# AlainSchoebi/semantic-bundle-adjustment-colmap

Hardware: AMD Instinct MI355X
Metric: residuals+Jacobians/sec and BA-iteration wall-time, 1k cams / 1M pts / 10M obs (higher is better)
Workload: dtype f64

## Files before the change

### semantic-bundle-adjustment-colmap_amd/csrc/context.h

```cpp
#pragma once

#include <hip/hip_runtime.h>
#include <rocblas/rocblas.h>
#include <rccl/rccl.h>

#include <map>
#include <string>
#include <vector>

#include "../../include/mi_ba.h"
#include "cholesky.h"
#include "device.h"
#include "setup.h"

namespace miba {

template <typename T>
struct DevArray {
  T* ptr = nullptr;
  size_t n = 0;
  size_t cap = 0;
  DevArray() = default;
  DevArray(const DevArray&) = delete;
  DevArray& operator=(const DevArray&) = delete;
  ~DevArray() { release(); }
  hipError_t alloc(size_t count) {
    if (ptr && count <= cap) {
      n = count;
      return hipSuccess;
    }
    release();
    n = count;
    if (count == 0) return hipSuccess;
    const hipError_t e = hipMalloc(&ptr, sizeof(T) * count);
    if (e == hipSuccess) cap = count;
    else ptr = nullptr;
    return e;
  }
  void release() {
    if (ptr) (void)hipFree(ptr);
    ptr = nullptr;
    n = 0;
    cap = 0;
  }
  size_t bytes() const { return sizeof(T) * n; }
};

struct SemanticState;
struct GsbaState;

struct KernelTimer {
  std::vector<std::pair<std::string, std::pair<hipEvent_t, hipEvent_t>>> pending;
  std::vector<hipEvent_t> pool;
  std::vector<hipEvent_t> borrowed;
  std::map<std::string, std::pair<double, int64_t>> totals;
};

}

struct mi_ba_context {
  mi_ba_options options;
  mi_ba_problem problem;
  miba::HostSetup setup;
  miba::DevProblem dev;
  hipStream_t stream = nullptr;
  int device = 0;

  std::vector<int64_t> block_obs;
  miba::DevArray<double2> obs_xy;
  miba::DevArray<uint32_t> obs_img, obs_pt;
  miba::DevArray<uint32_t> obs_ids, wave_pt0;
  miba::DevArray<uint32_t> img_flags, img_cam;
  miba::DevArray<uint8_t> cam_var, cam_model, pt_var;
  miba::DevArray<double> qt, cam, X;
  miba::DevArray<double> qt_c, cam_c, X_c;
  miba::DevArray<double> img_rec;
  miba::DevArray<uint32_t> cm_perm;
  miba::DevArray<uint32_t> cm_ptv;
  miba::DevArray<miba::DevTile> tiles;
  int ntiles = 0;
  miba::DevArray<uint32_t> img_tile_off, cam_tile_off, cam_tiles;
  miba::DevArray<double> tpart;
  bool det_sums = true;
  const miba::TileOwners* owners() const { return det_sums && tpart.ptr ? &owners_ : nullptr; }
  miba::TileOwners owners_{};
  miba::DevArray<miba::DevPoint> vpoints;
  int64_t npv = 0;
  int64_t nb_const = 0;
  miba::DevArray<uint32_t> pchunks;
  int npchunks = 0;
  miba::DevArray<double> sum_ws;
  int lin_overlap = 0;
  int lin_warm = 15;
  int lin_warm_conc = 0;
  int warm_unroll = 4;
  int warm_wgs = 2048;
  int lin_order = 0;
  hipStream_t lin_side = nullptr;
  hipEvent_t lin_ev[2] = {nullptr, nullptr};
  int sem_diag = 0;
  bool sem_deferred_box = false;
  int sem_prep_early = 0;
  int sem_dgrid = 24;
  int sem_dvar = 0;
  int sem_compact = 1;
  int sem_coarse = 2;
  int sem_variant = 6;

  miba::DevArray<double2> r;
  miba::DevArray<double> J;
  miba::DevArray<double> Jcm;
  bool jcm_stale = true;
  miba::DevArray<double> Vg;
  miba::DevArray<double> partial;
  int64_t npartial = 0;
  miba::DevArray<double> scale_p, diag_p, Vinv;
  miba::DevArray<double> pose_blk, cam_blk, bvec, udiag;
  miba::DevArray<double> scale_f, diag_f, lambda_f, prec_pose, prec_cam;
  miba::DevArray<double> cg_x, cg_r, cg_z, cg_p, cg_q, cg_w, dX;
  miba::DevArray<double> scalars;
  miba::DevArray<double> red;
  miba::DevArray<double> aux;
  double* host_scalars = nullptr;
  int32_t* host_info = nullptr;
  int host_info_cap = 0;
  bool chol_pending = false;
  int chol_leaves = 0;

  bool dense = false;
  rocblas_handle blas = nullptr;
  miba::DevArray<double> S;
  miba::DevArray<double> Linv, Z;
  miba::DevArray<miba::DevPairTile> ptiles;
  miba::DevArray<miba::DevPairTile> ptiles_blk;
  std::vector<miba::DevPairTile> ptiles_host;
  miba::DevArray<miba::DevPairTile> ptiles_xcd;
  int nptiles_xcd = 0;
  int schur_block = 8;
  miba::DevArray<int32_t> pslot;
  miba::DevArray<double> spart;
  miba::DevArray<uint4> pdest;
  miba::DevArray<uint8_t> pself;
  int npdest = 0;
  bool pflush_ok = false;
  miba::DevArray<uint4> podest, pochunk;
  miba::DevArray<uint32_t> poent;
  miba::DevArray<double> popart;
  int npodest = 0, npochunk = 0;
  miba::DevArray<uint2> pairs;
  miba::DevArray<uint2> pairs_pos;
  int nptiles = 0;
  miba::DevArray<int32_t> info;
  miba::CholConfig chol;
  bool fused_rhs = true;
  bool pcg_mf = false;
  miba::DevArray<double> Xcm;
  miba::DevArray<double2> obs_cm;
  bool xcm_stale = true;
  int pcg_jcm = 2;
  bool pn_chunks = true;
  bool pp_chunks = true;
  bool schur_overlap = false;
  hipStream_t lm_side = nullptr;
  hipEvent_t lm_ev[2] = {nullptr, nullptr};
  miba::CholWorkspace cholws;

  double fixed_cost = 0.0;
  miba::SemanticState* sem = nullptr;
  miba::GsbaState* gsba = nullptr;

  bool timing = false;
  miba::KernelTimer timer;
  bool solved = false;

  int rank = 0, world = 1;
  ncclComm_t comm = nullptr;
  bool comm_failed = false;
  int comm_timeout_ms = 300000;
  double comm_due = 0.0;
  int fail_factorizations = 0;
  int comm_stall_ms = 0;
  int* stall_flag = nullptr;
  mi_ba_host_allreduce_fn host_reduce = nullptr;
  void* host_reduce_user = nullptr;
  std::vector<double> reduce_buf;
  bool distributed() const { return world > 1 || comm != nullptr || comm_failed || host_reduce != nullptr; }
// ... 16 lines not shown
```

### semantic-bundle-adjustment-colmap_amd/csrc/runtime.hip

```cpp
#include <hip/hip_runtime.h>

#include <algorithm>
#include <atomic>
#include <chrono>
#include <condition_variable>
#include <memory>
#include <mutex>
#include <thread>
#include <cmath>
#include <cstdio>
#include <cstring>
#include <cstdlib>
#include <map>
#include <numeric>
#include <unordered_map>

#include "../../include/mi_ba.h"
#include "ba_math.h"
#include "cholesky.h"
#include "context.h"
#include "kernels.h"
#include "gsba.h"
#include "semantic.h"
#include "setup.h"
// ... 2018 lines not shown
  bool ok;
  {
    std::unique_lock<std::mutex> g(job->m);
    job->cv.wait_for(g, std::chrono::milliseconds(std::max(1, ctx->comm_timeout_ms)), [&] { return job->done; });
    ok = job->done && job->res == ncclSuccess && job->comm;
    if (!job->done) job->abandoned = true;
    if (ok) ctx->comm = job->comm;
  }
  if (!ok) return MI_BA_ERR_HIP;
  ctx->rank = rank;
  ctx->world = world;
  return reduce_fixed_cost(ctx);
}

mi_ba_status mi_ba_context_set_host_reducer(mi_ba_context* ctx, int32_t rank, int32_t world,
                                            mi_ba_host_allreduce_fn fn, void* user) {
  if (!ctx || !fn || world < 1 || rank < 0 || rank >= world) return MI_BA_ERR_INVALID_ARGUMENT;
  if (ctx->comm || ctx->host_reduce || ctx->solved) return MI_BA_ERR_STATE;
  ctx->host_reduce = fn;
  ctx->host_reduce_user = user;
  ctx->rank = rank;
  ctx->world = world;
  return reduce_fixed_cost(ctx);
}

#ifdef MI_BA_AB_VARIANTS
static bool ab_value(int, int) { return true; }
#else
static bool ab_value(int value, int product) { return value == product; }
#endif

mi_ba_status mi_ba_set_tuning(mi_ba_context* ctx, const char* key, int32_t value) {
  if (!ctx || !key) return MI_BA_ERR_INVALID_ARGUMENT;
  if (std::strcmp(key, "jacobian_variant") == 0 && value >= 0 && value <= 63 && ab_value(value, 0)) {
    ctx->dev.jvariant = value;
    return MI_BA_OK;
  }
  if (std::strcmp(key, "comm_timeout_ms") == 0 && value >= 1) {
    ctx->comm_timeout_ms = value;
    return MI_BA_OK;
  }
  if (std::strcmp(key, "test_fail_factorizations") == 0 && value >= 0 && value <= 1000) {
    ctx->fail_factorizations = value;
    return MI_BA_OK;
  }
  if (std::strcmp(key, "comm_stall_ms") == 0 && value >= 0 && value <= 60000) {
    ctx->comm_stall_ms = value;
    return MI_BA_OK;
  }
  if (std::strcmp(key, "linearize_warm_inputs") == 0 && value >= 0 && value <= 15) {
    ctx->lin_warm = value;
    return MI_BA_OK;
  }
  if (std::strcmp(key, "linearize_warm_concurrent") == 0 && value >= 0 && value <= 15 && ab_value(value, 0)) {
    ctx->lin_warm_conc = value;
    return MI_BA_OK;
  }
  if (std::strcmp(key, "warm_unroll") == 0 && (value == 4 || value == 8) && ab_value(value, 4)) {
    ctx->warm_unroll = value;
    return MI_BA_OK;
  }
  if (std::strcmp(key, "warm_workgroups") == 0 && value >= 0 && value <= 65536) {
    ctx->warm_wgs = value;
    return MI_BA_OK;
  }
  if (std::strcmp(key, "linearize_order") == 0 && (value == 0 || value == 1) && ab_value(value, 0)) {
    ctx->lin_order = value;
    return MI_BA_OK;
  }
  if (std::strcmp(key, "linearize_overlap") == 0 && value >= 0 && value <= 2 && ab_value(value, 0)) {
    ctx->lin_overlap = value;
    return MI_BA_OK;
  }
  if (std::strcmp(key, "semantic_prep_early") == 0 && (value == 0 || value == 1) && ab_value(value, 0)) {
    ctx->sem_prep_early = value;
    return MI_BA_OK;
  }
  if (std::strcmp(key, "semantic_deferred_variant") == 0 && value >= 0 && value <= 4 && ab_value(value, 0)) {
    ctx->sem_dvar = value;
    return MI_BA_OK;
  }
  if (std::strcmp(key, "semantic_deferred_grid") == 0 && value >= 1 && value <= 64) {
    ctx->sem_dgrid = value;
    return MI_BA_OK;
  }
  if (std::strcmp(key, "semantic_deferred_compact") == 0 && (value == 0 || value == 1)) {
    ctx->sem_compact = value;
    return MI_BA_OK;
  }
  if (std::strcmp(key, "semantic_flat_coarse") == 0 && value >= 0 && value <= 3) {
    ctx->sem_coarse = value;
    return MI_BA_OK;
  }
  if (std::strcmp(key, "semantic_diag") == 0 && value >= 0 && value <= 2) {
    ctx->sem_diag = value;
    return MI_BA_OK;
  }
  if (std::strcmp(key, "semantic_window_summary") == 0 && (value == 0 || value == 1)) {
    if (!ctx->sem) return value ? MI_BA_ERR_STATE : MI_BA_OK;
    return semantic_set_window_summary(ctx, value != 0);
  }
  if (std::strcmp(key, "semantic_label_planes") == 0 && (value == 0 || value == 1)) {
    if (!ctx->sem) return value ? MI_BA_ERR_STATE : MI_BA_OK;
    return semantic_set_label_planes(ctx, value != 0);
  }
  if (std::strcmp(key, "semantic_deferred_box") == 0 && (value == 0 || value == 1)) {
    ctx->sem_deferred_box = value != 0;
    return MI_BA_OK;
  }
  if (std::strcmp(key, "semantic_variant") == 0 && value >= 0 && value <= 6 && ab_value(value, 6)) {
    ctx->sem_variant = value;
    return MI_BA_OK;
  }
  if (std::strcmp(key, "schur_pairs_variant") == 0 && value >= 0 && value <= 9 &&
      (value == 0 || value == 4 || value == 6 || ab_value(value, 0))) {
    ctx->dev.svariant = value;
    return MI_BA_OK;
  }
  if (std::strcmp(key, "schur_self_one_load") == 0 && (value == 0 || value == 1) && ab_value(value, 1)) {
    ctx->dev.sself1 = value;
    return MI_BA_OK;
  }
  if (std::strcmp(key, "schur_z_image_order") == 0 && (value == 0 || value == 1) && ab_value(value, 0)) {
    ctx->dev.zorder = value;
    if (!value) {
      ctx->pairs_pos.release();
      return MI_BA_OK;
    }
    return ctx->pairs.n ? build_pairs_pos(ctx, nullptr) : MI_BA_OK;
  }
  if (std::strcmp(key, "fblock_variant") == 0 && value >= 0 && value <= 2 && ab_value(value, 0)) {
    ctx->dev.fvariant = value;
    return MI_BA_OK;
  }
  if (std::strcmp(key, "schur_block_images") == 0 && value >= 1) {
    ctx->schur_block = value;
    return ctx->ptiles_host.empty() ? MI_BA_OK : order_block_tiles(ctx);
  }
  if (std::strcmp(key, "cholesky_panel") == 0 && (value == 0 || (value >= 64 && value <= 4096))) {
    ctx->chol.panel = value;
    return MI_BA_OK;
  }
  if (std::strcmp(key, "cholesky_head_panel") == 0 && (value == 0 || (value >= 64 && value <= 1024))) {
    ctx->chol.head_panel = value;
    return MI_BA_OK;
  }
  if (std::strcmp(key, "cholesky_head_cols") == 0 && value >= 0) {
    ctx->chol.head_cols = value;
    return MI_BA_OK;
  }
  if (std::strcmp(key, "cholesky_tail_panel") == 0 && (value == 0 || (value >= 64 && value <= 1024))) {
    ctx->chol.tail_panel = value;
    return MI_BA_OK;
  }
  if (std::strcmp(key, "cholesky_tail_cols") == 0 && value >= 0) {
    ctx->chol.tail_cols = value;
    return MI_BA_OK;
  }
  if (std::strcmp(key, "cholesky_lookahead") == 0 && (value == 0 || value == 1)) {
    ctx->chol.lookahead = value != 0;
    return MI_BA_OK;
  }
  if (std::strcmp(key, "cholesky_head_own_diag") == 0 && (value == 0 || value == 2 || value == 6) &&
      ab_value(value, 0)) {
    ctx->chol.head_own = (int)value;
    return MI_BA_OK;
// ... 257 lines not shown
```

### semantic-bundle-adjustment-colmap_amd/csrc/semantic.h

```cpp
#pragma once

#include <hip/hip_runtime.h>

#include <cstdint>
#include <functional>

#include "../../include/mi_ba.h"
#include "ba_math.h"
#include "context.h"

namespace miba {

struct SemSample {
  double pc1[3];
  float label1;
  uint32_t pair;
};

struct SemTile {
  uint32_t pair, start, count, pad;
};

struct SemPair {
  uint32_t i, j;
  uint32_t var1, var2;
  uint32_t start, count;
};

struct SlotInfo {
  uint64_t off, toff;
  int32_t H, W, TW, pad;
};

struct SemanticState {
  std::vector<int32_t> img_h, img_w;
  std::vector<SlotInfo> slots_host;
  DevArray<SlotInfo> slots;
  int64_t npix = 0;
  int64_t ntile = 0;
  int max_plane = 0, max_tiles = 0;
  double depth_threshold = 2.0;
  double rel_step = 1e-3;
  int step = 1;
  std::vector<uint8_t> has_raster;
  int64_t ns = 0;
  int npairs = 0;
  std::vector<SemPair> pairs_host;
  std::vector<int32_t> sample_pixel_host;
  DevArray<SemSample> samples;
  DevArray<SemPair> pairs;
  DevArray<float2> dl;
  int nslots = 0;
  DevArray<float4> wsum;
  bool use_wsum = false;
  DevArray<uint8_t> lab8;
  DevArray<float2> dtile;
  DevArray<float> pal;
  bool use_lp = false;
  DevArray<uint32_t> raster_slot;
  DevArray<double> r;
  DevArray<int32_t> status;
  DevArray<double> J;
  DevArray<double> pconst;
  bool samples_valid = false;
  DevArray<double> pair_blk;
  DevArray<double> partial;
  int64_t npartial = 0;
  DevArray<SemTile> tiles;
  int ntiles = 0;
  int model_tiles[kNumModels + 1] = {};
  DevArray<uint32_t> pair_cnt;
  DevArray<uint32_t> dlist;
  DevArray<uint2> chunks;
  DevArray<uint2> dchunks;
  DevArray<uint32_t> dcount;
  int n_cu = 256;
  int model_chunks[kNumModels + 1] = {};
  DevArray<unsigned long long> dmask;
  DevArray<uint32_t> pair_tile0, pair_chunk0;
  DevArray<double> cpart;
  DevArray<uint32_t> img_pairs_off, img_pairs;
  DevArray<uint2> sblk;
  DevArray<uint32_t> sblk_off, sblk_ent;
  int nsblk = 0;
  DevArray<double> mpart;
};

mi_ba_status semantic_create(mi_ba_context* ctx, const mi_ba_semantic* sem);
void semantic_destroy(mi_ba_context* ctx);
mi_ba_status semantic_linearize(mi_ba_context* ctx, double* d_cost, bool write_samples,
                                hipStream_t deferred_stream = nullptr, hipEvent_t flat_done = nullptr,
                                hipEvent_t timer_start = nullptr, const double* other_partial = nullptr,
                                int64_t other_n = 0, double* other_out = nullptr, double* other_scratch = nullptr,
                                const std::function<mi_ba_status()>& after_flat = nullptr,
                                hipEvent_t prep_done = nullptr);
mi_ba_status semantic_pair_prep(mi_ba_context* ctx, hipStream_t stream);
mi_ba_status semantic_export(mi_ba_context* ctx, int32_t image1, int32_t image2, int64_t* count, int32_t* pixels,
                             int32_t* status, double* error, double* world);
mi_ba_status semantic_set_window_summary(mi_ba_context* ctx, bool on);
mi_ba_status semantic_set_label_planes(mi_ba_context* ctx, bool on);
void semantic_cost(mi_ba_context* ctx, const double* qt, const double* cam, double* d_cost);
void semantic_add_fblock(mi_ba_context* ctx);
void semantic_add_gradient(mi_ba_context* ctx, double* g);
void semantic_schur_product(mi_ba_context* ctx, const double* x, double* y);
void semantic_add_dense(mi_ba_context* ctx, double* S);
void semantic_model_cost(mi_ba_context* ctx, const double* df, double* d_out);

}
```

### semantic-bundle-adjustment-colmap_amd/csrc/semantic.hip

```cpp
#include <hip/hip_runtime.h>

#include <map>

#include <algorithm>
#include <cmath>
#include <cstring>
#include <type_traits>

#include "ba_math.h"
#include "kernels.h"
#include "semantic.h"

namespace miba {

namespace {

constexpr double kMinStep = 1.4901161193847656e-08;

struct SemArgs {
  const SemSample* samples;
  const SemPair* pairs;
  const double* qt;
  const double* cam;
  const uint32_t* img_cam;
// ... 1379 lines not shown
                                                              const uint32_t* __restrict__ ccount,
                                                              const PairConst* __restrict__ pcs,
                                                              const uint32_t* __restrict__ pair_cnt,
                                                              const uint32_t* __restrict__ dlist,
                                                              const uint32_t* __restrict__ pair_chunk0,
                                                              double* __restrict__ cpart,
                                                              double* __restrict__ J_out, int write_samples,
                                                              int32_t* __restrict__ status_out = nullptr) {
  __shared__ double sJ[64 * kSemRow];
  __shared__ float2 sbox[BOX ? 64 * 9 : 1];
  const uint32_t nch = ccount ? *ccount : blockIdx.x + 1;
  const uint32_t stride = ccount ? gridDim.x : 1u;
  for (uint32_t ci = blockIdx.x; ci < nch; ci += stride) {
  const uint2 ch = chunks[ci];
  const uint32_t cnt = pair_cnt[ch.x];
  if (ch.y >= cnt) continue;
  const PairConst* __restrict__ P = pcs + ch.x;
  const SemArgs a = with_pair(ak, P);
  const int lane = threadIdx.x;
  const uint32_t k = ch.y + lane;
  const uint32_t pstart = a.pairs[ch.x].start;
  const float2* dl2 = a.dl + P->roff;
  const double* K2 = P->K2;
  double rowv[kSemRow];
#pragma unroll
  for (int q = 0; q < kSemRow; ++q) rowv[q] = 0.0;
  if (k < cnt) {
    const int64_t n = (int64_t)pstart + dlist[pstart + k];
    const SemSample smp = a.samples[n];
    Centre c;
    centre_eval<M, FAST>(a, P, smp, K2, dl2, c);
    double Jt[12];
    bool redone;
    if constexpr (BOX) {
      FlatBox fb;
      if (flat_box<M>(P, c, K2, fb)) {
        float2* mine = sbox + 9 * lane;
#pragma unroll
        for (int q = 0; q < 9; ++q) mine[q] = dl2[flat_index(a, fb, true, q)];
        redone = stencil_full<M, FAST, NB>(a, P, c, smp, K2, dl2, Jt, mine, &fb);
      } else {
        redone = stencil_full<M, FAST, NB>(a, P, c, smp, K2, dl2, Jt);
      }
    } else {
      redone = stencil_full<M, FAST, NB>(a, P, c, smp, K2, dl2, Jt);
    }
    if ((write_samples & 4) && status_out && redone) status_out[n] += 0x10000;
    if (write_samples) {
      double2* jo = reinterpret_cast<double2*>(J_out + 12 * n);
#pragma unroll
      for (int m = 0; m < 6; ++m) jo[m] = make_double2(Jt[2 * m], Jt[2 * m + 1]);
    }
    double rho[3];
    loss_eval(a.loss_type, a.loss_scale, c.r * c.r, rho);
    const double sc = sqrt(a.weight * rho[1]);
#pragma unroll
    for (int m = 0; m < 12; ++m) rowv[m] = Jt[m] * sc;
    rowv[12] = c.r * sc;
  }
#pragma unroll
  for (int q = 0; q < kSemRow; ++q) sJ[lane * kSemRow + q] = rowv[q];
  __syncthreads();
  const int rows = min(64, (int)(cnt - ch.y));
#pragma unroll
  for (int h = 0; h < 2; ++h) {
    const int e = lane + 64 * h;
    if (e < kPairVals) {
      int ca, cb;
      if (e < 78) {
        int a_ = 0, rem = e;
        while (rem >= 12 - a_) { rem -= 12 - a_; ++a_; }
        ca = a_;
        cb = a_ + rem;
      } else {
        ca = e - 78;
        cb = 12;
      }
      double acc = 0.0;
      for (int q = 0; q < rows; ++q) acc += sJ[q * kSemRow + ca] * sJ[q * kSemRow + cb];
      cpart[((size_t)pair_chunk0[ch.x] + ch.y / 64) * kPairVals + e] = acc;
    }
  }
  __syncthreads();
  }
}

__global__ __launch_bounds__(256) void deferred_order_kernel(const unsigned long long* __restrict__ dmask,
                                                             const uint32_t* __restrict__ pair_tile0,
                                                             const SemPair* __restrict__ pairs,
                                                             uint32_t* __restrict__ pair_cnt,
                                                             uint32_t* __restrict__ dlist) {
  __shared__ uint32_t sc[256];
  const int p = blockIdx.x, tid = threadIdx.x;
  const SemPair pr = pairs[p];
  const uint32_t words = (pr.count + 63) / 64;
  const unsigned long long* mk = dmask + (size_t)pair_tile0[p] * (kBlock / 64);
  uint32_t base = 0;
  for (uint32_t w0 = 0; w0 < words; w0 += 256) {
    const uint32_t w = w0 + tid;
    const unsigned long long m = w < words ? mk[w] : 0ull;
    const uint32_t c = (uint32_t)__popcll(m);
    sc[tid] = c;
    __syncthreads();
    for (int off = 1; off < 256; off <<= 1) {
      const uint32_t v = tid >= off ? sc[tid - off] : 0u;
      __syncthreads();
      sc[tid] += v;
      __syncthreads();
    }
    uint32_t o = base + sc[tid] - c;
    for (unsigned long long r = m; r; r &= r - 1) dlist[pr.start + o++] = 64 * w + (uint32_t)__ffsll((long long)r) - 1;
    base += sc[255];
    __syncthreads();
  }
  if (tid == 0) pair_cnt[p] = base;
}

__global__ __launch_bounds__(128) void pair_reduce_kernel(const uint32_t* __restrict__ pair_cnt,
                                                          const uint32_t* __restrict__ pair_chunk0,
                                                          const double* __restrict__ cpart,
                                                          double* __restrict__ pair_blk) {
  const int p = blockIdx.x, e = threadIdx.x;
  if (e >= kPairVals) return;
  const uint32_t nch = (pair_cnt[p] + 63) / 64;
  const double* c = cpart + (size_t)pair_chunk0[p] * kPairVals + e;
  double v = 0.0;
  for (uint32_t j = 0; j < nch; ++j) v += c[(size_t)j * kPairVals];
  pair_blk[(size_t)p * kPairStride + e] = v;
}

struct ModelRanges {
  int b[kNumModels + 1];
};

__global__ __launch_bounds__(256) void deferred_compact_kernel(const uint2* __restrict__ chunks, int nchunks,
                                                               const uint32_t* __restrict__ pair_cnt, ModelRanges mr,
                                                               uint2* __restrict__ out, uint32_t* __restrict__ cnt) {
  __shared__ uint32_t swc[4][kNumModels];
  __shared__ uint32_t sbase[kNumModels];
  const int i = blockIdx.x * 256 + threadIdx.x;
  const int lane = threadIdx.x & 63, wv = threadIdx.x >> 6;
  const bool valid = i < nchunks;
  uint2 ch = make_uint2(0u, 0u);
  int m = 0;
  bool live = false;
  if (valid) {
    ch = chunks[i];
    live = ch.y < pair_cnt[ch.x];
    while (m + 1 < kNumModels && i >= mr.b[m + 1]) ++m;
  }
  uint32_t rank = 0;
#pragma unroll
  for (int mm = 0; mm < kNumModels; ++mm) {
    const unsigned long long sel = __ballot(live && m == mm);
    if (lane == 0) swc[wv][mm] = (uint32_t)__popcll(sel);
    if (live && m == mm) rank = (uint32_t)__popcll(sel & ((1ull << lane) - 1ull));
  }
  __syncthreads();
  if (threadIdx.x < kNumModels) {
    const uint32_t tot = swc[0][threadIdx.x] + swc[1][threadIdx.x] + swc[2][threadIdx.x] + swc[3][threadIdx.x];
    sbase[threadIdx.x] = tot ? atomicAdd(cnt + threadIdx.x, tot) : 0u;
  }
  __syncthreads();
  if (live) {
    uint32_t off = sbase[m];
    for (int w = 0; w < wv; ++w) off += swc[w][m];
// ... 422 lines not shown
      const SemPair& pr = S->pairs_host[k];
      const int m = hs.cam_model[p->image_camera[pr.j]];
      for (uint32_t off = 0; off < pr.count; off += 64) per[m].push_back(make_uint2((uint32_t)k, off));
    }
    S->model_chunks[0] = 0;
    for (int m = 0; m < kNumModels; ++m) {
      chunks.insert(chunks.end(), per[m].begin(), per[m].end());
      S->model_chunks[m + 1] = (int)chunks.size();
    }
  }
  if (S->pair_cnt.alloc(std::max(1, S->npairs)) || S->dlist.alloc(std::max<int64_t>(1, S->ns)) ||
      S->chunks.alloc(std::max<size_t>(1, chunks.size())) || S->dchunks.alloc(std::max<size_t>(1, chunks.size())) ||
      S->dcount.alloc(kNumModels))
    return MI_BA_ERR_OUT_OF_MEMORY;
  {
    const int np = S->npairs;
    std::vector<uint32_t> tile0(std::max(1, np), 0), chunk0(std::max(1, np), 0);
    for (size_t k = tiles.size(); k-- > 0;) tile0[tiles[k].pair] = (uint32_t)k;
    std::vector<uint32_t> nchk(std::max(1, np), 0);
    for (const uint2& c : chunks) ++nchk[c.x];
    for (size_t k = chunks.size(); k-- > 0;) chunk0[chunks[k].x] = (uint32_t)k;
    for (int k = 0; k < np; ++k) {
      const SemPair& pr = S->pairs_host[k];
      const uint32_t nt = (pr.count + kBlock - 1) / kBlock;
      for (uint32_t j = 0; j < nt; ++j)
        if (tiles[tile0[k] + j].pair != (uint32_t)k || tiles[tile0[k] + j].start != pr.start + j * kBlock)
          return MI_BA_ERR_HIP;
      for (uint32_t j = 0; j < nchk[k]; ++j)
        if (chunks[chunk0[k] + j].x != (uint32_t)k || chunks[chunk0[k] + j].y != 64 * j) return MI_BA_ERR_HIP;
    }
    std::vector<uint32_t> ipo(I + 1, 0), ip;
    for (int k = 0; k < np; ++k) {
      ++ipo[S->pairs_host[k].i + 1];
      ++ipo[S->pairs_host[k].j + 1];
    }
    for (int i = 0; i < I; ++i) ipo[i + 1] += ipo[i];
    ip.resize(ipo[I]);
    {
      std::vector<uint32_t> pos(ipo.begin(), ipo.end() - 1);
      for (int k = 0; k < np; ++k) {
        ip[pos[S->pairs_host[k].i]++] = (uint32_t)k << 1;
        ip[pos[S->pairs_host[k].j]++] = (uint32_t)k << 1 | 1u;
      }
    }
    std::map<std::pair<uint32_t, uint32_t>, std::vector<uint32_t>> blocks;
    for (int k = 0; k < np; ++k) {
      const SemPair& pr = S->pairs_host[k];
      blocks[{pr.i, pr.i}].push_back((uint32_t)k << 1);
      blocks[{pr.j, pr.j}].push_back((uint32_t)k << 1 | 1u);
      if (pr.i < pr.j)
        blocks[{pr.i, pr.j}].push_back((uint32_t)k << 1);
      else
        blocks[{pr.j, pr.i}].push_back((uint32_t)k << 1 | 1u);
    }
    std::vector<uint2> sb;
    std::vector<uint32_t> so(1, 0), se;
    for (auto& b : blocks) {
      sb.push_back(make_uint2(b.first.first, b.first.second));
      se.insert(se.end(), b.second.begin(), b.second.end());
      so.push_back((uint32_t)se.size());
    }
    S->nsblk = (int)sb.size();
    if (S->dmask.alloc(std::max<size_t>(1, tiles.size()) * (kBlock / 64)) || S->pair_tile0.alloc(tile0.size()) ||
        S->pair_chunk0.alloc(chunk0.size()) || S->cpart.alloc(std::max<size_t>(1, chunks.size()) * kPairVals) ||
        S->img_pairs_off.alloc(ipo.size()) || S->img_pairs.alloc(std::max<size_t>(1, ip.size())) ||
        S->sblk.alloc(std::max<size_t>(1, sb.size())) || S->sblk_off.alloc(so.size()) ||
        S->sblk_ent.alloc(std::max<size_t>(1, se.size())) || S->mpart.alloc((std::max(1, np) + 63) / 64))
      return MI_BA_ERR_OUT_OF_MEMORY;
    if (hipMemcpy(S->pair_tile0.ptr, tile0.data(), tile0.size() * 4, hipMemcpyHostToDevice) ||
        hipMemcpy(S->pair_chunk0.ptr, chunk0.data(), chunk0.size() * 4, hipMemcpyHostToDevice) ||
        hipMemcpy(S->img_pairs_off.ptr, ipo.data(), ipo.size() * 4, hipMemcpyHostToDevice) ||
        (!ip.empty() && hipMemcpy(S->img_pairs.ptr, ip.data(), ip.size() * 4, hipMemcpyHostToDevice)) ||
        (!sb.empty() && hipMemcpy(S->sblk.ptr, sb.data(), sb.size() * sizeof(uint2), hipMemcpyHostToDevice)) ||
        hipMemcpy(S->sblk_off.ptr, so.data(), so.size() * 4, hipMemcpyHostToDevice) ||
        (!se.empty() && hipMemcpy(S->sblk_ent.ptr, se.data(), se.size() * 4, hipMemcpyHostToDevice)))
      return MI_BA_ERR_HIP;
  }
  {
    int dev = 0, ncu = 0;
    if (hipGetDevice(&dev) != hipSuccess || hipDeviceGetAttribute(&ncu, hipDeviceAttributeMultiprocessorCount, dev) ||
        ncu <= 0)
      ncu = 256;
    S->n_cu = ncu;
  }
  if (!chunks.empty() && hipMemcpy(S->chunks.ptr, chunks.data(), chunks.size() * sizeof(uint2), hipMemcpyHostToDevice))
    return MI_BA_ERR_HIP;
  if (S->samples.alloc(S->ns) || S->pairs.alloc(S->npairs) || S->raster_slot.alloc(I) ||
      S->slots.alloc(std::max<size_t>(1, S->slots_host.size())) ||
      S->dl.alloc(std::max<size_t>(1, (size_t)S->npix)) || S->r.alloc(S->ns) ||
      S->status.alloc(S->ns) || S->J.alloc(12 * S->ns) ||
      S->pair_blk.alloc((size_t)kPairStride * std::max(1, S->npairs)) || S->tiles.alloc(tiles.size()) ||
      S->pconst.alloc(sizeof(PairConst) / sizeof(double) * std::max(1, S->npairs)))
    return MI_BA_ERR_OUT_OF_MEMORY;
  S->npartial = std::max<int64_t>({(int64_t)tiles.size(), (S->ns + kBlock - 1) / kBlock, (int64_t)1});
  if (S->partial.alloc(S->npartial)) return MI_BA_ERR_OUT_OF_MEMORY;
  if ((S->ns && hipMemcpy(S->samples.ptr, samples.data(), S->ns * sizeof(SemSample), hipMemcpyHostToDevice)) ||
      (S->npairs &&
       hipMemcpy(S->pairs.ptr, S->pairs_host.data(), S->npairs * sizeof(SemPair), hipMemcpyHostToDevice)) ||
      (I && hipMemcpy(S->raster_slot.ptr, slot_u.data(), I * 4, hipMemcpyHostToDevice)) ||
      (!S->slots_host.empty() && hipMemcpy(S->slots.ptr, S->slots_host.data(), S->slots_host.size() * sizeof(SlotInfo),
                                           hipMemcpyHostToDevice)) ||
      (!tiles.empty() &&
       hipMemcpy(S->tiles.ptr, tiles.data(), tiles.size() * sizeof(SemTile), hipMemcpyHostToDevice)))
    return MI_BA_ERR_HIP;
  std::vector<float2> buf((size_t)S->max_plane);
  for (size_t s = 0; s < slot_images.size(); ++s) {
    const int j = slot_images[s];
    const size_t plane = (size_t)img_h[j] * img_w[j];
    const float* d = sem->depth + img_off[j];
    const float* l = sem->label + img_off[j];
    for (size_t k = 0; k < plane; ++k) buf[k] = make_float2(d[k], l[k]);
    if (hipMemcpy(S->dl.ptr + S->slots_host[s].off, buf.data(), plane * sizeof(float2), hipMemcpyHostToDevice))
      return MI_BA_ERR_HIP;
  }
  mi_ba_status st = semantic_set_label_planes(ctx, true);
  if (st == MI_BA_ERR_HIP) return st;
  if (!S->use_lp && semantic_set_window_summary(ctx, true) == MI_BA_ERR_HIP) return MI_BA_ERR_HIP;
  return MI_BA_OK;
}

mi_ba_status semantic_export(mi_ba_context* ctx, int32_t image1, int32_t image2, int64_t* count, int32_t* pixels,
                             int32_t* status, double* error, double* world) {
  SemanticState* S = ctx->sem;
  const int I = ctx->problem.num_images;
  if (!S || !count || image1 < 0 || image1 >= I || image2 < 0 || image2 >= I || image1 == image2)
    return MI_BA_ERR_INVALID_ARGUMENT;
  const int H1 = S->img_h[image1], W1 = S->img_w[image1];
  const int nx = (W1 + S->step - 1) / S->step, ny = (H1 + S->step - 1) / S->step;
  const int64_t n = (int64_t)nx * ny;
  *count = n;
  if (!pixels) return MI_BA_OK;
  if (!status || !error || !world) return MI_BA_ERR_INVALID_ARGUMENT;
  if (!S->has_raster[image1] || !S->has_raster[image2]) return MI_BA_ERR_UNSUPPORTED;
  if (n == 0) return MI_BA_OK;
  DevArray<int32_t> d_pix, d_st;
  DevArray<double> d_err, d_w;
  if (d_pix.alloc(4 * n) || d_st.alloc(n) || d_err.alloc(n) || d_w.alloc(3 * n)) return MI_BA_ERR_OUT_OF_MEMORY;
  SemArgs a = make_args(ctx, ctx->dev.qt, ctx->dev.cam);
  hipLaunchKernelGGL(semantic_export_kernel, dim3((unsigned)((n + kBlock - 1) / kBlock)), dim3(kBlock), 0, ctx->stream,
                     a, (uint32_t)image1, (uint32_t)image2, S->step, nx, n, d_pix.ptr, d_st.ptr, d_err.ptr, d_w.ptr);
  if (hipGetLastError() != hipSuccess ||
      hipMemcpyAsync(pixels, d_pix.ptr, 16 * n, hipMemcpyDeviceToHost, ctx->stream) != hipSuccess ||
      hipMemcpyAsync(status, d_st.ptr, 4 * n, hipMemcpyDeviceToHost, ctx->stream) != hipSuccess ||
      hipMemcpyAsync(error, d_err.ptr, 8 * n, hipMemcpyDeviceToHost, ctx->stream) != hipSuccess ||
      hipMemcpyAsync(world, d_w.ptr, 24 * n, hipMemcpyDeviceToHost, ctx->stream) != hipSuccess ||
      hipStreamSynchronize(ctx->stream) != hipSuccess)
    return MI_BA_ERR_HIP;
  return MI_BA_OK;
}

mi_ba_status semantic_set_window_summary(mi_ba_context* ctx, bool on) {
  SemanticState* S = ctx->sem;
  if (!S) return MI_BA_ERR_STATE;
  if (on && !S->wsum.ptr) {
    const int64_t n = S->npix;
    if (n > 0) {
      if (S->wsum.alloc((size_t)n)) {
        (void)hipGetLastError();
        S->use_wsum = false;
        return MI_BA_ERR_OUT_OF_MEMORY;
      }
      hipLaunchKernelGGL(window_summary_kernel, dim3((unsigned)((S->max_plane + 255) / 256), (unsigned)S->nslots),
                         dim3(256), 0, ctx->stream, S->dl.ptr, S->slots.ptr, S->wsum.ptr);
      if (hipGetLastError() != hipSuccess) return MI_BA_ERR_HIP;
    }
  }
// ... 36 lines not shown
  unsigned ov = 0;
  if (hipGetLastError() != hipSuccess || hipMemcpyAsync(hk, keys.ptr, sizeof(hk), hipMemcpyDeviceToHost, s) ||
      hipMemcpyAsync(&ov, overflow.ptr, sizeof(ov), hipMemcpyDeviceToHost, s) || hipStreamSynchronize(s))
    return MI_BA_ERR_HIP;
  if (ov) {
    S->lab8.release();
    S->dtile.release();
    S->pal.release();
    return MI_BA_OK;
  }
  float hp[256];
  for (int k = 0; k < 256; ++k) {
    const uint32_t b = (uint32_t)(hk[k] & 0xffffffffull);
    std::memcpy(&hp[k], &b, 4);
  }
  hipLaunchKernelGGL(label_index_kernel, dim3(g), dim3(256), 0, s, S->dl.ptr, n, keys.ptr, S->lab8.ptr);
  hipLaunchKernelGGL(depth_tile_kernel, dim3((unsigned)((S->max_tiles + 255) / 256), (unsigned)S->nslots), dim3(256),
                     0, s, S->dl.ptr, S->slots.ptr, S->dtile.ptr);
  if (hipGetLastError() != hipSuccess || hipMemcpyAsync(S->pal.ptr, hp, sizeof(hp), hipMemcpyHostToDevice, s) ||
      hipStreamSynchronize(s))
    return MI_BA_ERR_HIP;
  S->use_lp = true;
  return MI_BA_OK;
}

void semantic_destroy(mi_ba_context* ctx) {
  if (!ctx->sem) return;
  delete ctx->sem;
  ctx->sem = nullptr;
}

mi_ba_status semantic_pair_prep(mi_ba_context* ctx, hipStream_t stream) {
  SemanticState* S = ctx->sem;
  if (!S || S->ns == 0 || S->npairs == 0) return MI_BA_OK;
  SemArgs a = make_args(ctx, ctx->dev.qt, ctx->dev.cam);
  PairConst* pcs = reinterpret_cast<PairConst*>(S->pconst.ptr);
  hipLaunchKernelGGL(semantic_pair_prep_kernel, dim3((S->npairs + 1) / 2), dim3(64), 0, stream, S->pairs.ptr,
                     S->npairs, a.qt, a.cam, a.img_cam, a.img_flags, a.raster_slot, a.slots, a.rel_step, pcs,
                     S->pair_blk.ptr,
                     kPairStride, ctx->sem_variant == 6 ? S->pair_cnt.ptr : nullptr,
                     ctx->sem_variant == 6 ? S->dcount.ptr : nullptr, kNumModels);
  return hipGetLastError() == hipSuccess ? MI_BA_OK : MI_BA_ERR_HIP;
}

mi_ba_status semantic_linearize(mi_ba_context* ctx, double* d_cost, bool write_samples, hipStream_t deferred_stream,
                                hipEvent_t flat_done, hipEvent_t timer_start, const double* other_partial,
                                int64_t other_n, double* other_out, double* other_scratch,
                                const std::function<mi_ba_status()>& after_flat, hipEvent_t prep_done) {
  SemanticState* S = ctx->sem;
  hipStream_t s = ctx->stream;
  S->samples_valid = write_samples;
  if (S->ns == 0) {
    if (S->npairs && hipMemsetAsync(S->pair_blk.ptr, 0, S->pair_blk.bytes(), s) != hipSuccess) return MI_BA_ERR_HIP;
    if (other_partial) launch_sum(other_partial, other_n, other_out, s, other_scratch);
    return MI_BA_OK;
  }
  SemArgs a = make_args(ctx, ctx->dev.qt, ctx->dev.cam);
  PairConst* pcs = reinterpret_cast<PairConst*>(S->pconst.ptr);
  hipEvent_t stop;
  timer_begin_after(ctx, "semantic_jacobian", timer_start, &stop);
  if (prep_done) {
    if (hipStreamWaitEvent(s, prep_done, 0) != hipSuccess) return MI_BA_ERR_HIP;
  } else {
    const mi_ba_status st = semantic_pair_prep(ctx, s);
    if (st != MI_BA_OK) return st;
  }
  const bool split = deferred_stream != nullptr && ctx->sem_variant == 6;
  if (ctx->sem_variant == 6) {
    const int ws = write_samples ? 1 | (ctx->sem_diag ? 2 : 0) | (ctx->sem_diag == 2 ? 4 : 0) : 0;
    auto deferred = [&](hipStream_t ds) -> mi_ba_status {
      hipLaunchKernelGGL(deferred_order_kernel, dim3(S->npairs), dim3(256), 0, ds, S->dmask.ptr, S->pair_tile0.ptr,
                         S->pairs.ptr, S->pair_cnt.ptr, S->dlist.ptr);
      const int nall = S->model_chunks[kNumModels];
      const bool compact = ctx->sem_compact != 0;
      if (nall > 0 && compact) {
        ModelRanges mr;
        for (int m = 0; m <= kNumModels; ++m) mr.b[m] = S->model_chunks[m];
        hipLaunchKernelGGL(deferred_compact_kernel, dim3((unsigned)((nall + 255) / 256)), dim3(256), 0, ds,
                           S->chunks.ptr, nall, S->pair_cnt.ptr, mr, S->dchunks.ptr, S->dcount.ptr);
      }
      for (int model = 0; model < kNumModels; ++model) {
        const int c0 = S->model_chunks[model], nc = S->model_chunks[model + 1] - c0;
        if (S->model_tiles[model + 1] == S->model_tiles[model] || nc == 0) continue;
        const int grid = compact ? std::min(nc, std::max(1, ctx->sem_dgrid) * S->n_cu) : nc;
        const uint2* list = (compact ? S->dchunks.ptr : S->chunks.ptr) + c0;
        const uint32_t* count = compact ? S->dcount.ptr + model : nullptr;
        dispatch_model(model, [&](auto m) {
          constexpr int M = decltype(m)::value;
          if (ctx->sem_deferred_box)
            hipLaunchKernelGGL((semantic_deferred_kernel<M, true, 4, true>), dim3(grid), dim3(64), 0, ds, a, list,
                               count, pcs, S->pair_cnt.ptr, S->dlist.ptr, S->pair_chunk0.ptr, S->cpart.ptr, S->J.ptr,
                               ws, S->status.ptr);
#ifdef MI_BA_AB_VARIANTS
          else if (ctx->sem_dvar == 1)
            hipLaunchKernelGGL((semantic_deferred_kernel<M, true, 2>), dim3(grid), dim3(64), 0, ds, a, list, count,
                               pcs, S->pair_cnt.ptr, S->dlist.ptr, S->pair_chunk0.ptr, S->cpart.ptr, S->J.ptr, ws,
                               S->status.ptr);
          else if (ctx->sem_dvar == 2)
            hipLaunchKernelGGL((semantic_deferred_kernel<M, true, 2, false, 5>), dim3(grid), dim3(64), 0, ds, a,
                               list, count, pcs, S->pair_cnt.ptr, S->dlist.ptr, S->pair_chunk0.ptr, S->cpart.ptr, S->J.ptr,
                               ws, S->status.ptr);
          else if (ctx->sem_dvar == 3)
            hipLaunchKernelGGL((semantic_deferred_kernel<M, true, 4, false, 5>), dim3(grid), dim3(64), 0, ds, a,
                               list, count, pcs, S->pair_cnt.ptr, S->dlist.ptr, S->pair_chunk0.ptr, S->cpart.ptr, S->J.ptr,
                               ws, S->status.ptr);
          else if (ctx->sem_dvar == 4)
            hipLaunchKernelGGL((semantic_deferred_kernel<M, true, 2, false, 6>), dim3(grid), dim3(64), 0, ds, a,
                               list, count, pcs, S->pair_cnt.ptr, S->dlist.ptr, S->pair_chunk0.ptr, S->cpart.ptr, S->J.ptr,
                               ws, S->status.ptr);
#endif
          else
            hipLaunchKernelGGL((semantic_deferred_kernel<M, true, 4>), dim3(grid), dim3(64), 0, ds, a, list, count,
                               pcs, S->pair_cnt.ptr, S->dlist.ptr, S->pair_chunk0.ptr, S->cpart.ptr, S->J.ptr, ws,
                               S->status.ptr);
        });
      }
      hipLaunchKernelGGL(pair_reduce_kernel, dim3(S->npairs), dim3(128), 0, ds, S->pair_cnt.ptr, S->pair_chunk0.ptr,
                         S->cpart.ptr, S->pair_blk.ptr);
      return MI_BA_OK;
    };
    for (int model = 0; model < kNumModels; ++model) {
      const int t0 = S->model_tiles[model], nt = S->model_tiles[model + 1] - t0;
      if (nt == 0) continue;
      dispatch_model(model, [&](auto m) {
        constexpr int M = decltype(m)::value;
        auto launch = [&](auto ws_, auto lp_, auto coarse_) {
          hipLaunchKernelGGL((semantic_flat_kernel<M, true, decltype(ws_)::value, decltype(lp_)::value,
                                                   decltype(coarse_)::value>),
                             dim3(nt), dim3(kBlock), 0, s, a, S->tiles.ptr + t0, pcs,
                             S->dmask.ptr + (size_t)t0 * (kBlock / 64), S->partial.ptr + t0, S->r.ptr, S->status.ptr,
                             S->J.ptr, ws);
        };
        using T = std::true_type;
        using F = std::false_type;
        using C0 = std::integral_constant<int, 0>;
        using C1 = std::integral_constant<int, 1>;
        using C2 = std::integral_constant<int, 2>;
        using C3 = std::integral_constant<int, 3>;
        auto pick = [&](auto ws_, auto lp_) {
          if (ctx->sem_coarse == 3) launch(ws_, lp_, C3{});
          else if (ctx->sem_coarse == 2) launch(ws_, lp_, C2{});
          else if (ctx->sem_coarse == 1) launch(ws_, lp_, C1{});
          else launch(ws_, lp_, C0{});
        };
        if (a.lab8)
          pick(F{}, T{});
        else if (a.wsum)
          pick(T{}, F{});
        else
          pick(F{}, F{});
      });
    }
    if (after_flat) {
      const mi_ba_status st = after_flat();
      if (st != MI_BA_OK) return st;
    }
    if (split) {
      if (hipEventRecord(flat_done, s) != hipSuccess || hipStreamWaitEvent(deferred_stream, flat_done, 0) != hipSuccess)
        return MI_BA_ERR_HIP;
      const mi_ba_status st = deferred(deferred_stream);
      if (st != MI_BA_OK) return st;
    } else {
      const mi_ba_status st = deferred(s);
      if (st != MI_BA_OK) return st;
    }
  }
#ifdef MI_BA_AB_VARIANTS
  for (int model = 0; model < kNumModels && ctx->sem_variant != 6; ++model) {
    const int t0 = S->model_tiles[model], nt = S->model_tiles[model + 1] - t0;
    if (nt == 0) continue;
    dispatch_model(model, [&](auto m) {
      constexpr int M = decltype(m)::value;
// ... 83 lines not shown
```

Before: 19.04 billion.

## Split deferred semantic stencil across four waves per 64-sample chunk

Adds a 256-thread deferred semantic kernel in which each of four wavefronts evaluates one stencil group (a subset of the 12 Jacobian columns) for the same 64 samples. Partial columns go through shared memory, then a 64-row block-level reduction forms the pair normal-equation partials. This is meant to cut per-thread serial stencil work and add latency hiding. In exchange it recomputes the centre geometry in every wave and adds LDS traffic and barriers. Grid size now defaults to occupancy-derived blocks per CU instead of the fixed grid multiplier.

Measured after the change: 19.55 billion, median of 6. 2.7% higher.

```diff
diff --git a/semantic-bundle-adjustment-colmap_amd/csrc/context.h b/semantic-bundle-adjustment-colmap_amd/csrc/context.h
--- a/semantic-bundle-adjustment-colmap_amd/csrc/context.h
+++ b/semantic-bundle-adjustment-colmap_amd/csrc/context.h
@@ -102,6 +102,8 @@
   bool sem_deferred_box = false;
   int sem_prep_early = 0;
   int sem_dgrid = 24;
+  bool sem_dgrid_set = false;
+  int sem_dwaves = 4;
   int sem_dvar = 0;
   int sem_compact = 1;
   int sem_coarse = 2;
diff --git a/semantic-bundle-adjustment-colmap_amd/csrc/runtime.hip b/semantic-bundle-adjustment-colmap_amd/csrc/runtime.hip
--- a/semantic-bundle-adjustment-colmap_amd/csrc/runtime.hip
+++ b/semantic-bundle-adjustment-colmap_amd/csrc/runtime.hip
@@ -2124,6 +2124,11 @@
   }
   if (std::strcmp(key, "semantic_deferred_grid") == 0 && value >= 1 && value <= 64) {
     ctx->sem_dgrid = value;
+    ctx->sem_dgrid_set = true;
+    return MI_BA_OK;
+  }
+  if (std::strcmp(key, "semantic_deferred_waves") == 0 && (value == 1 || value == 4)) {
+    ctx->sem_dwaves = value;
     return MI_BA_OK;
   }
   if (std::strcmp(key, "semantic_deferred_compact") == 0 && (value == 0 || value == 1)) {
diff --git a/semantic-bundle-adjustment-colmap_amd/csrc/semantic.h b/semantic-bundle-adjustment-colmap_amd/csrc/semantic.h
--- a/semantic-bundle-adjustment-colmap_amd/csrc/semantic.h
+++ b/semantic-bundle-adjustment-colmap_amd/csrc/semantic.h
@@ -75,6 +75,7 @@
   DevArray<uint2> dchunks;
   DevArray<uint32_t> dcount;
   int n_cu = 256;
+  int dwaves_blocks[kNumModels] = {};
   int model_chunks[kNumModels + 1] = {};
   DevArray<unsigned long long> dmask;
   DevArray<uint32_t> pair_tile0, pair_chunk0;
diff --git a/semantic-bundle-adjustment-colmap_amd/csrc/semantic.hip b/semantic-bundle-adjustment-colmap_amd/csrc/semantic.hip
--- a/semantic-bundle-adjustment-colmap_amd/csrc/semantic.hip
+++ b/semantic-bundle-adjustment-colmap_amd/csrc/semantic.hip
@@ -1485,6 +1485,188 @@
     }
   }
   __syncthreads();
+  }
+}
+
+template <int M>
+__device__ __forceinline__ void centre_geometry(const PairConst* __restrict__ P, const SemSample& smp,
+                                                const double* K2, Centre& c) {
+  double rot[3];
+  unit_quat_rotate(P->uqi, smp.pc1, rot);
+  c.pw[0] = rot[0] + P->ti[0];
+  c.pw[1] = rot[1] + P->ti[1];
+  c.pw[2] = rot[2] + P->ti[2];
+  double rot2[3];
+  unit_quat_rotate(P->u2, c.pw, rot2);
+  c.p2[0] = rot2[0] + P->t2[0];
+  c.p2[1] = rot2[1] + P->t2[1];
+  c.p2[2] = rot2[2] + P->t2[2];
+  c.pc.valid = false;
+  c.pc.px = c.pc.py = 0;
+  c.pc.depth = c.pc.label = 0.f;
+  c.st = 0;
+  c.r = 0.0;
+  c.mag = fabs(smp.pc1[0]) + fabs(smp.pc1[1]) + fabs(smp.pc1[2]) + fabs(P->t1[0]) + fabs(P->t1[1]) +
+          fabs(P->t1[2]) + fabs(c.pw[0]) + fabs(c.pw[1]) + fabs(c.pw[2]) + fabs(P->t2[0]) + fabs(P->t2[1]) +
+          fabs(P->t2[2]);
+  c.w[0] = smp.pc1[0] - P->t1[0];
+  c.w[1] = smp.pc1[1] - P->t1[1];
+  c.w[2] = smp.pc1[2] - P->t1[2];
+  c.exk = margin_model_term<M>(K2, c.p2, c.mag);
+}
+
+template <int M, int GRP>
+__device__ __forceinline__ bool stencil_group(const SemArgs& a, const PairConst* __restrict__ P, const Centre& c,
+                                              const SemSample& smp, const double* K2, const float2* dl2,
+                                              double col[3]) {
+  constexpr int n = (GRP == 0 || GRP == 2) ? 4 : 3;
+  constexpr int m0 = GRP == 0 ? 0 : (GRP == 1 ? 4 : (GRP == 2 ? 7 : 11));
+  const uint32_t mask = GRP == 1 ? P->mask1 : (GRP == 3 ? P->mask2 : 0u);
+  col[0] = col[1] = col[2] = 0.0;
+  const PixelCache none = {0, 0, 0.f, 0.f, false};
+  double fp[4], fm[4];
+  const bool ok = stencil_step<M, true, GRP, 4>(a, P, m0, 0, n, c.w, c.pw, c.p2, c.mag, smp.label1, K2, dl2, 0, c.exk,
+                                                fp, fm);
+  if (ok) {
+#pragma unroll
+    for (int j = 0; j < n; ++j) {
+      const double jm = (fp[j] - fm[j]) * P->ood[m0 + j];
+      if constexpr (GRP == 0 || GRP == 2) {
+        const double* pj = P->pj[(GRP == 0 ? 0 : 4) + j];
+#pragma unroll
+        for (int q = 0; q < 3; ++q) col[q] = col[q] + jm * pj[q];
+      } else {
+        const double v = ((mask >> j) & 1u) ? 0.0 : jm;
+#pragma unroll
+        for (int q = 0; q < 3; ++q) col[q] = q == j ? v : col[q];
+      }
+    }
+    return false;
+  }
+#pragma unroll 1
+  for (int k = 0; k < n; ++k) {
+    const int m = m0 + k;
+    double f2[2] = {0.0, 0.0};
+#pragma unroll 1
+    for (int sg = 0; sg < 2; ++sg) {
+      const double f = stencil_point<M, true, GRP>(a, P, 2 * m + sg, k, c.w, c.pw, c.p2, c.mag, smp.pc1, smp.label1,
+                                                   K2, dl2, none, c.exk);
+      f2[0] = sg == 0 ? f : f2[0];
+      f2[1] = sg == 1 ? f : f2[1];
+    }
+    const double jm = (f2[0] - f2[1]) * P->ood[m];
+    if constexpr (GRP == 0 || GRP == 2) {
+      const double* pj = P->pj[(GRP == 0 ? 0 : 4) + k];
+#pragma unroll
+      for (int q = 0; q < 3; ++q) col[q] = col[q] + jm * pj[q];
+    } else {
+      const double v = ((mask >> k) & 1u) ? 0.0 : jm;
+#pragma unroll
+      for (int q = 0; q < 3; ++q) col[q] = q == k ? v : col[q];
+    }
+  }
+  return true;
+}
+
+template <int M>
+__global__ __launch_bounds__(256) void semantic_deferred_waves_kernel(SemArgs ak, const uint2* __restrict__ chunks,
+                                                                     const uint32_t* __restrict__ ccount,
+                                                                     const PairConst* __restrict__ pcs,
+                                                                     const uint32_t* __restrict__ pair_cnt,
+                                                                     const uint32_t* __restrict__ dlist,
+                                                                     const uint32_t* __restrict__ pair_chunk0,
+                                                                     double* __restrict__ cpart,
+                                                                     double* __restrict__ J_out, int write_samples,
+                                                                     int32_t* __restrict__ status_out = nullptr) {
+  __shared__ double sraw[64 * 12];
+  __shared__ double ssc[64], srs[64];
+  __shared__ double sJ[64 * kSemRow];
+  __shared__ uint8_t sredo[4 * 64];
+  const int tid = threadIdx.x, lane = tid & 63;
+  const int wv = __builtin_amdgcn_readfirstlane(tid >> 6);
+  const uint32_t nch = ccount ? *ccount : blockIdx.x + 1;
+  const uint32_t stride = ccount ? gridDim.x : 1u;
+  for (uint32_t ci = blockIdx.x; ci < nch; ci += stride) {
+    const uint2 ch = chunks[ci];
+    const uint32_t cnt = pair_cnt[ch.x];
+    if (ch.y >= cnt) continue;
+    const PairConst* __restrict__ P = pcs + ch.x;
+    const SemArgs a = with_pair(ak, P);
+    const uint32_t k = ch.y + lane;
+    const uint32_t pstart = a.pairs[ch.x].start;
+    const float2* dl2 = a.dl + P->roff;
+    const double* K2 = P->K2;
+    double col[3] = {0.0, 0.0, 0.0};
+    bool redone = false;
+    int64_t n = 0;
+    if (k < cnt) {
+      n = (int64_t)pstart + dlist[pstart + k];
+      const SemSample smp = a.samples[n];
+      Centre c;
+      if (wv == 0) {
+        centre_geometry<M>(P, smp, K2, c);
+        if (P->var1) redone = stencil_group<M, 0>(a, P, c, smp, K2, dl2, col);
+      } else if (wv == 1) {
+        centre_geometry<M>(P, smp, K2, c);
+        if (P->var1) redone = stencil_group<M, 1>(a, P, c, smp, K2, dl2, col);
+      } else if (wv == 2) {
+        centre_geometry<M>(P, smp, K2, c);
+        if (P->var2) redone = stencil_group<M, 2>(a, P, c, smp, K2, dl2, col);
+      } else {
+        centre_eval<M, true>(a, P, smp, K2, dl2, c);
+        if (P->var2) redone = stencil_group<M, 3>(a, P, c, smp, K2, dl2, col);
+        double rho[3];
+        loss_eval(a.loss_type, a.loss_scale, c.r * c.r, rho);
+        const double sc = sqrt(a.weight * rho[1]);
+        ssc[lane] = sc;
+        srs[lane] = c.r * sc;
+      }
+    }
+#pragma unroll
+    for (int q = 0; q < 3; ++q) sraw[lane * 12 + 3 * wv + q] = col[q];
+    sredo[wv * 64 + lane] = redone ? 1 : 0;
+    __syncthreads();
+    if (tid < 64) {
+      double rowv[kSemRow];
+#pragma unroll
+      for (int q = 0; q < kSemRow; ++q) rowv[q] = 0.0;
+      if (k < cnt) {
+        double Jt[12];
+#pragma unroll
+        for (int m = 0; m < 12; ++m) Jt[m] = sraw[lane * 12 + m];
+        if ((write_samples & 4) && status_out && (sredo[lane] | sredo[64 + lane] | sredo[128 + lane] | sredo[192 + lane]))
+          status_out[n] += 0x10000;
+        if (write_samples) {
+          double2* jo = reinterpret_cast<double2*>(J_out + 12 * n);
+#pragma unroll
+          for (int m = 0; m < 6; ++m) jo[m] = make_double2(Jt[2 * m], Jt[2 * m + 1]);
+        }
+        const double sc = ssc[lane];
+#pragma unroll
+        for (int m = 0; m < 12; ++m) rowv[m] = Jt[m] * sc;
+        rowv[12] = srs[lane];
+      }
+#pragma unroll
+      for (int q = 0; q < kSemRow; ++q) sJ[lane * kSemRow + q] = rowv[q];
+    }
+    __syncthreads();
+    const int rows = min(64, (int)(cnt - ch.y));
+    if (tid < kPairVals) {
+      const int e = tid;
+      int ca, cb;
+      if (e < 78) {
+        int a_ = 0, rem = e;
+        while (rem >= 12 - a_) { rem -= 12 - a_; ++a_; }
+        ca = a_;
+        cb = a_ + rem;
+      } else {
+        ca = e - 78;
+        cb = 12;
+      }
+      double acc = 0.0;
+      for (int q = 0; q < rows; ++q) acc += sJ[q * kSemRow + ca] * sJ[q * kSemRow + cb];
+      cpart[((size_t)pair_chunk0[ch.x] + ch.y / 64) * kPairVals + e] = acc;
+    }
   }
 }
 
@@ -2073,6 +2255,17 @@
         ncu <= 0)
       ncu = 256;
     S->n_cu = ncu;
+    for (int model = 0; model < kNumModels; ++model) {
+      dispatch_model(model, [&](auto m) {
+        constexpr int M = decltype(m)::value;
+        int nb = 0;
+        if (hipOccupancyMaxActiveBlocksPerMultiprocessor(&nb, semantic_deferred_waves_kernel<M>, 256, 0) !=
+                hipSuccess ||
+            nb <= 0)
+          nb = 4;
+        S->dwaves_blocks[model] = nb;
+      });
+    }
   }
   if (!chunks.empty() && hipMemcpy(S->chunks.ptr, chunks.data(), chunks.size() * sizeof(uint2), hipMemcpyHostToDevice))
     return MI_BA_ERR_HIP;
@@ -2275,12 +2468,23 @@
       for (int model = 0; model < kNumModels; ++model) {
         const int c0 = S->model_chunks[model], nc = S->model_chunks[model + 1] - c0;
         if (S->model_tiles[model + 1] == S->model_tiles[model] || nc == 0) continue;
-        const int grid = compact ? std::min(nc, std::max(1, ctx->sem_dgrid) * S->n_cu) : nc;
+        const bool waves4 = ctx->sem_dwaves == 4 && !ctx->sem_deferred_box
+#ifdef MI_BA_AB_VARIANTS
+                            && ctx->sem_dvar == 0
+#endif
+            ;
+        const int per_cu = waves4 && !ctx->sem_dgrid_set ? std::max(1, S->dwaves_blocks[model])
+                                                         : std::max(1, ctx->sem_dgrid);
+        const int grid = compact ? std::min(nc, per_cu * S->n_cu) : nc;
         const uint2* list = (compact ? S->dchunks.ptr : S->chunks.ptr) + c0;
         const uint32_t* count = compact ? S->dcount.ptr + model : nullptr;
         dispatch_model(model, [&](auto m) {
           constexpr int M = decltype(m)::value;
-          if (ctx->sem_deferred_box)
+          if (waves4)
+            hipLaunchKernelGGL((semantic_deferred_waves_kernel<M>), dim3(grid), dim3(256), 0, ds, a, list, count,
+                               pcs, S->pair_cnt.ptr, S->dlist.ptr, S->pair_chunk0.ptr, S->cpart.ptr, S->J.ptr, ws,
+                               S->status.ptr);
+          else if (ctx->sem_deferred_box)
             hipLaunchKernelGGL((semantic_deferred_kernel<M, true, 4, true>), dim3(grid), dim3(64), 0, ds, a, list,
                                count, pcs, S->pair_cnt.ptr, S->dlist.ptr, S->pair_chunk0.ptr, S->cpart.ptr, S->J.ptr,
                                ws, S->status.ptr);
```
